# hassony2/homan

Measured on AMD Instinct MI355X. Metric: optimisation iters/sec (30-frame 256^2 clip), higher is better.
Workload: dtype f32

## Files before the change

### homan_amd/csrc/raster_common.h

```cpp
#pragma once
#include "hm_common.h"
#include <type_traits>

#define HM_TILE 8
#define HM_STILE 16
#define RASTER_WAVES 4
#define STAGE_DW 20

typedef int hm_v2i __attribute__((ext_vector_type(2)));
typedef unsigned hm_v4u __attribute__((ext_vector_type(4)));
#ifndef RASTER_NT_STORES
#define RASTER_NT_STORES 0
#endif
__device__ __forceinline__ void hm_out_store(float* p, float v)
{
#if RASTER_NT_STORES
    __builtin_nontemporal_store(v, p);
#else
    *p = v;
#endif
}
__device__ __forceinline__ void hm_out_store2(int* p, int a, int b)
{
#if RASTER_NT_STORES
// ... 14 lines not shown
}

struct FaceBox {
    unsigned short x0m, y0, x1, y1;
};

__device__ __forceinline__ float topix(float v, int is)
{
    float a = v * (float)is;
    a = a + (float)is;
    a = a - 1.0f;
    return 0.5f * a;
}
__device__ __forceinline__ bool backside(const float* f)
{
    return (f[7] - f[1]) * (f[3] - f[0]) < (f[4] - f[1]) * (f[6] - f[0]);
}
__device__ __forceinline__ void wave_sync()
{
    __builtin_amdgcn_fence(__ATOMIC_ACQ_REL, "wavefront");
    __builtin_amdgcn_wave_barrier();
}

#define SR_MAX 64
__host__ __device__ __forceinline__ int hm_sr_shift(int is) { return is <= 512 ? 6 : 7; }

__device__ __forceinline__ int hm_wave_scan_incl(int v)
{
    v += __builtin_amdgcn_update_dpp(0, v, 0x111, 0xf, 0xf, false);
    v += __builtin_amdgcn_update_dpp(0, v, 0x112, 0xf, 0xf, false);
    v += __builtin_amdgcn_update_dpp(0, v, 0x114, 0xf, 0xf, false);
    v += __builtin_amdgcn_update_dpp(0, v, 0x118, 0xf, 0xf, false);
    v += __builtin_amdgcn_update_dpp(0, v, 0x142, 0xa, 0xf, false);
    v += __builtin_amdgcn_update_dpp(0, v, 0x143, 0xc, 0xf, false);
    return v;
}

__device__ __forceinline__ float rlane(float v, int l)
{
    return __builtin_bit_cast(float, __builtin_amdgcn_readlane(__builtin_bit_cast(int, v), l));
}

__device__ __forceinline__ unsigned spread8(unsigned x)
{
    x = (x | (x << 4)) & 0x0f0fu;
    x = (x | (x << 2)) & 0x3333u;
    x = (x | (x << 1)) & 0x5555u;
    return x;
}
__device__ __forceinline__ long hm_plane_at(int b, int ty, int tx, int combo, int T)
{
    return ((((long)b * T + ty) * T + tx) * 4 + combo) * 16;
}
__device__ __forceinline__ unsigned long long hm_plane_word64(const unsigned short* __restrict__ planes, int b, int is,
                                                              int axis, int pl, int d0, int k)
{
    const int T = is / 16;
    unsigned long long w = 0ull;
#pragma unroll
    for (int j = 0; j < 4; ++j) {
        unsigned v;
        if (axis) {
            const int t = is - 1 - d0;
            v = planes[hm_plane_at(b, t >> 4, 4 * k + j, pl, T) + (t & 15)];
        } else {
            v = planes[hm_plane_at(b, T - 1 - (4 * k + j), d0 >> 4, 2 + pl, T) + (d0 & 15)];
        }
        w |= (unsigned long long)v << (16 * j);
    }
    return w;
}
struct Ballots4 { unsigned long long s0, s1, s2, s3; };
__device__ __forceinline__ void emit_planes(const Ballots4 cov, const Ballots4 nb, const Ballots4 pb, int b, int B, int is,
                                            int tx, int ty, int lane, unsigned short* __restrict__ planes)
{
    const int l = lane & 15, pl = (lane >> 4) & 1, hi = l >> 1, sub = l & 1;
    unsigned long long b0, b1;
    unsigned word;
    const Ballots4 g = pl == 0 ? nb : pb;
    if (lane < 32) {
        const unsigned long long c0 = sub ? cov.s2 : cov.s0, c1 = sub ? cov.s3 : cov.s1;
        const unsigned long long g0 = sub ? g.s2 : g.s0, g1 = sub ? g.s3 : g.s1;
        b0 = pl == 0 ? (~c0 & g0) : (c0 & g0);
        b1 = pl == 0 ? (~c1 & g1) : (c1 & g1);
        const unsigned a = (unsigned)(b0 >> (8 * hi)) & 0xffu, o = (unsigned)(b1 >> (8 * hi)) & 0xffu;
        word = spread8(a) | (spread8(o) << 1);
    } else {
        const unsigned long long c0 = sub ? cov.s1 : cov.s0, c1 = sub ? cov.s3 : cov.s2;
        const unsigned long long g0 = sub ? g.s1 : g.s0, g1 = sub ? g.s3 : g.s2;
        b0 = pl == 0 ? (~c0 & g0) : (c0 & g0);
        b1 = pl == 0 ? (~c1 & g1) : (c1 & g1);
        const unsigned k0 = (unsigned)((((b0 >> hi) & 0x0101010101010101ull) * 0x8040201008040201ull) >> 56);
        const unsigned k1 = (unsigned)((((b1 >> hi) & 0x0101010101010101ull) * 0x8040201008040201ull) >> 56);
        word = (spread8(k0) << 1) | spread8(k1);
    }
    const unsigned p2 = (word & 0xffffu) | ((unsigned)__builtin_amdgcn_update_dpp(0, (int)word, 0x101, 0xf, 0xf, false) << 16);
    const unsigned q2 = (unsigned)__builtin_amdgcn_update_dpp(0, (int)p2, 0x102, 0xf, 0xf, false);
    const unsigned r2 = (unsigned)__builtin_amdgcn_update_dpp(0, (int)p2, 0x104, 0xf, 0xf, false);
    const unsigned s2 = (unsigned)__builtin_amdgcn_update_dpp(0, (int)q2, 0x104, 0xf, 0xf, false);
    if ((lane & 7) == 0) hm_out_store4(planes + hm_plane_at(b, ty, tx, 0, is / 16) + lane, p2, q2, r2, s2);
}

__device__ __forceinline__ bool hm_ts_enabled(const unsigned int* __restrict__ flag_word)
{
    return flag_word && ((flag_word[0] >> 8) & 1u);
}
__device__ __forceinline__ void hm_ts_store(unsigned long long* __restrict__ slots, long unit, int which, unsigned long long t)
{
    __builtin_nontemporal_store(t, slots + 2 * unit + which);
}

__device__ __forceinline__ void sil_reduce_frame(int b, const float* __restrict__ partials, int ntiles,
                                                 const float* __restrict__ keep_sum, float* __restrict__ frame_rec,
                                                 float* __restrict__ out, float* __restrict__ frame_out, int clip_len,
                                                 int out_stride)
{
    __shared__ float red[16];
    __shared__ int s_flag;
    float sq = 0.f, in = 0.f, un = 0.f;
    for (int t = threadIdx.x; t < ntiles; t += blockDim.x) {
        const float4 p = *reinterpret_cast<const float4*>(partials + ((long)b * ntiles + t) * 4);
        sq += p.x; in += p.y; un += p.z;
    }
    sq = hm_block_sum(sq, red);
    in = hm_block_sum(in, red);
    un = hm_block_sum(un, red);
    if (threadIdx.x == 0) { hm_partial_store(frame_rec + 4 * b, sq); hm_partial_store(frame_rec + 4 * b + 1, in / (un + 1e-6f)); }
    if (frame_out && threadIdx.x == 0) { frame_out[2 * b] = sq; frame_out[2 * b + 1] = in / (un + 1e-6f); }
    if (!out) return;
    const int clip = b / clip_len;
    float* crec = frame_rec + 4L * clip * clip_len;
    if (hm_last_block(reinterpret_cast<unsigned int*>(crec + 3), clip_len, &s_flag)) {
        const float total_sq = hm_last_block_sum(crec, clip_len, 4, red);
        const float iou_sum = hm_last_block_sum(crec + 1, clip_len, 4, red);
        if (threadIdx.x == 0) {
            out[(long)clip * out_stride] = (total_sq / keep_sum[clip]) / (float)clip_len;
            out[(long)clip * out_stride + 1] = iou_sum / (float)clip_len;
        }
    }
}

struct SweepFace {
    int bf, b, off, flags;
    float px[3], py[3];
    unsigned short cum[12];
};
#define SWEEP_PASS_FACES 16
#ifndef SWEEP_USHIFT
#define SWEEP_USHIFT 8
#endif
#define SWEEP_UNIT (1 << SWEEP_USHIFT)
#define SWEEP_TRIPS (SWEEP_UNIT / 64)
#define SWEEP_TBATCH (SWEEP_TRIPS < 4 ? SWEEP_TRIPS : 4)
struct SweepItem { float x, c0, c1; int base0, base1, nb0, fn, meta; };
struct SweepList {
    SweepFace* tab; int* offs; unsigned int* ufirst; unsigned int* tickets; float* upart;
    unsigned long long* cnt; unsigned int* done; unsigned long long* total;
    int ucap, slot_cap;
};

struct SweepSrc { int d1; float g; int owner; };
#define SWEEP_CUMW 16

template <bool W32> struct HmOff { typedef long t; };
template <> struct HmOff<true> { typedef unsigned t; };
template <bool W32, class T>
__device__ __forceinline__ T* hm_at(T* __restrict__ base, typename HmOff<W32>::t i)
{
    typedef typename std::conditional<std::is_const<T>::value, const char, char>::type byte_t;
    if (W32) return reinterpret_cast<T*>(reinterpret_cast<byte_t*>(base) + (unsigned)(i * (unsigned)sizeof(T)));
    return base + i;
}
```

### homan_amd/csrc/raster_lines.hip

```cpp
#include "raster_ws.h"

__global__ __launch_bounds__(256) void k_bwd_masks(const float* __restrict__ gin, int mode,
                                                   const float* __restrict__ upstream,
                                                   const float* __restrict__ keep_sum, int B, int S,
                                                   const unsigned short* __restrict__ alpha16,
                                                   float* __restrict__ gimg, unsigned short* __restrict__ planes,
                                                   int clip_len)
{
    if (mode == 1 && upstream[0] > 0.0f) return;
    const int w = threadIdx.x >> 6, lane = threadIdx.x & 63;
    const int is = 2 * S, tiles_x = S / HM_TILE, ntiles = tiles_x * tiles_x;
    const int tile = blockIdx.x * 4 + w, b = blockIdx.y;
    if (tile >= ntiles) return;
    const int ty = tile / tiles_x, tx = tile % tiles_x;
    const int rr = lane >> 3, cc = lane & 7;
    const int r = ty * HM_TILE + rr, c = tx * HM_TILE + cc;
    const long po = ((long)b * S + r) * S + c;
    unsigned long long cq[4];
#pragma unroll
    for (int dy = 0; dy < 2; ++dy) {
        const unsigned aw = alpha16[(((long)b * (is / 16) + ty) * (is / 16) + tx) * 16 + 2 * rr + dy];
#pragma unroll
        for (int dx = 0; dx < 2; ++dx) cq[2 * dy + dx] = __ballot((aw >> (2 * cc + dx)) & 1u);
    }
// ... 137 lines not shown
            atomicExch(sl.done, 0u);
        }
    }
}


#ifndef LINES_NL
#define LINES_NL 2
#endif
#ifdef LINES_REVERSED
#define LINES_BLK(i, n) ((n) - 1 - (i))
#else
#define LINES_BLK(i, n) (i)
#endif
template <bool W32>
__global__ __launch_bounds__(256) void k_bwd_lines(const unsigned short* __restrict__ planes,
                                                   const float* __restrict__ gimg, const float* __restrict__ dimg,
                                                   int mode, const float* __restrict__ upstream,
                                                   const float* __restrict__ keep_sum,
                                                   const int* __restrict__ idx_map, int B, int S,
                                                   SweepSrc* __restrict__ srcs, uint4* __restrict__ lrec,
                                                   int ncomp, int fpt, const float* __restrict__ faces9,
                                                   const FaceBox* __restrict__ boxes,
                                                   const unsigned char* __restrict__ owned, int F,
                                                   double* __restrict__ parts, SweepList sl, int clip_len,
                                                   unsigned short* __restrict__ lsum, int nred,
                                                   const float* __restrict__ red_partials, float* __restrict__ frame_rec,
                                                   float* __restrict__ loss_out, int out_stride,
                                                   const unsigned int* __restrict__ ts_flag,
                                                   unsigned long long* __restrict__ ts_slots)
{
    HM_CHAIN_KERNEL();
    const unsigned long long ts_t0 = (unsigned long long)wall_clock64();
    const bool ts_on = hm_ts_enabled(ts_flag) && threadIdx.x == 0;
    if (ts_on) hm_ts_store(ts_slots, blockIdx.x, 0, ts_t0);
    const int blk = (int)blockIdx.x;
    __shared__ unsigned long long s_w[16][LINES_NL][SWEEP_CUMW];
    __shared__ int s_ex[16][LINES_NL][SWEEP_CUMW];
    if (blk < ncomp) {
        sweep_compact(blk, ncomp, fpt, faces9, boxes, owned, B, F, 2 * S, parts, sl, clip_len);
        if (ts_on) hm_ts_store(ts_slots, blockIdx.x, 1, (unsigned long long)wall_clock64());
        return;
    }
    if (blk < ncomp + nred) {
        sil_reduce_frame(blk - ncomp, red_partials, (S / 8) * (S / 8), keep_sum, frame_rec, loss_out, nullptr, clip_len,
                         out_stride);
        if (ts_on) hm_ts_store(ts_slots, blockIdx.x, 1, (unsigned long long)wall_clock64());
        return;
    }
    typedef typename HmOff<W32>::t OFF;
    const int l = threadIdx.x & 15, grp = threadIdx.x >> 4;
    const bool ts_row = l == 0 && hm_ts_enabled(ts_flag);
    const int is = 2 * S, wpl = is / 64, T = is / 16;
    const unsigned Lw = (unsigned)(LINES_BLK(blk - ncomp - nred, (int)gridDim.x - ncomp - nred)) * (16u * LINES_NL);
    const bool valid = Lw < 4u * (unsigned)B * (unsigned)is;
    const unsigned fr = Lw / (unsigned)is;
    const int d00 = (int)(Lw - fr * (unsigned)is) + grp * LINES_NL, b = (int)(fr % (unsigned)B), pa = (int)(fr / (unsigned)B);
    const OFF L0 = (OFF)Lw + (OFF)(grp * LINES_NL);
    const int axis = pa & 1, pl = pa >> 1;
    unsigned long long mine[LINES_NL];
#pragma unroll
    for (int j = 0; j < LINES_NL; ++j) mine[j] = 0ull;
    if (valid && l < wpl) {
        unsigned long long raw[4];
#pragma unroll
        for (int jj = 0; jj < 4; ++jj) {
            OFF at;
            if (axis) {
                const int t = is - 1 - d00 - (LINES_NL - 1);
                at = ((((OFF)b * T + (t >> 4)) * T + (4 * l + jj)) * 4 + pl) * 16 + (t & 15);
            } else {
                at = ((((OFF)b * T + (T - 1 - (4 * l + jj))) * T + (d00 >> 4)) * 4 + (2 + pl)) * 16 + (d00 & 15);
            }
#if LINES_NL == 4
            raw[jj] = *reinterpret_cast<const unsigned long long*>(hm_at<W32>(planes, at));
#elif LINES_NL == 2
            raw[jj] = *reinterpret_cast<const unsigned int*>(hm_at<W32>(planes, at));
#else
            raw[jj] = *hm_at<W32>(planes, at);
#endif
        }
#pragma unroll
        for (int j = 0; j < LINES_NL; ++j) {
            const int sel = axis ? LINES_NL - 1 - j : j;
#pragma unroll
            for (int jj = 0; jj < 4; ++jj) mine[j] |= ((raw[jj] >> (16 * sel)) & 0xffffull) << (16 * jj);
        }
    }
    bool any = false;
#pragma unroll
    for (int j = 0; j < LINES_NL; ++j) {
        const OFF L = L0 + j;
        const int d0 = d00 + j;
        const int c = __popcll(mine[j]);
        int incl = c;
        incl += __builtin_amdgcn_update_dpp(0, incl, 0x111, 0xf, 0xf, false);
        incl += __builtin_amdgcn_update_dpp(0, incl, 0x112, 0xf, 0xf, false);
        incl += __builtin_amdgcn_update_dpp(0, incl, 0x114, 0xf, 0xf, false);
        incl += __builtin_amdgcn_update_dpp(0, incl, 0x118, 0xf, 0xf, false);
        const int excl = incl - c;
        if (valid && l < wpl) *hm_at<W32>(lrec, L * wpl + l) = make_uint4((unsigned)mine[j], (unsigned)(mine[j] >> 32), (unsigned)excl, 0u);
        int lo = mine[j] ? 64 * l + __builtin_ctzll(mine[j]) : 0xffff, hi = mine[j] ? 64 * l + 64 - __builtin_clzll(mine[j]) : 0;
        lo = min(lo, __builtin_amdgcn_update_dpp(0xffff, lo, 0x111, 0xf, 0xf, false)); hi = max(hi, __builtin_amdgcn_update_dpp(0, hi, 0x111, 0xf, 0xf, false));
        lo = min(lo, __builtin_amdgcn_update_dpp(0xffff, lo, 0x112, 0xf, 0xf, false)); hi = max(hi, __builtin_amdgcn_update_dpp(0, hi, 0x112, 0xf, 0xf, false));
        lo = min(lo, __builtin_amdgcn_update_dpp(0xffff, lo, 0x114, 0xf, 0xf, false)); hi = max(hi, __builtin_amdgcn_update_dpp(0, hi, 0x114, 0xf, 0xf, false));
        lo = min(lo, __builtin_amdgcn_update_dpp(0xffff, lo, 0x118, 0xf, 0xf, false)); hi = max(hi, __builtin_amdgcn_update_dpp(0, hi, 0x118, 0xf, 0xf, false));
        const unsigned wm = (unsigned)(__ballot(mine[j] != 0ull) >> (16 * (grp & 3))) & 0xffffu;
        if (valid && l == 15)
            *reinterpret_cast<uint2*>(hm_at<W32>(lsum, ((((OFF)b * 2 + axis) * is + d0) * 2 + pl) * 4)) =
                make_uint2((unsigned)lo | ((unsigned)hi << 16), wm);
        any = any || wm != 0u;
        s_w[grp][j][l] = mine[j];
        s_ex[grp][j][l] = excl;
    }
    wave_sync();
    if (!valid || !any) {
        if (ts_row) atomicMax(ts_slots + 2 * blockIdx.x + 1, (unsigned long long)wall_clock64());
        return;
    }
    const bool from_dimg = mode == 2 || (mode == 1 && upstream[0] > 0.0f);
    const float* gi = (from_dimg ? dimg : gimg) + (long)b * S * S;
    const float gs = from_dimg ? upstream[0] * 2.0f : 0.f, ks = from_dimg ? keep_sum[b / clip_len] : 1.f;
    const float up4 = (mode == 4 || mode == 5) ? upstream[b] * 2.0f : 0.f;
    const int* idx = idx_map + (long)b * is * is;
    const float* gfull = gimg + (long)b * is * is;
#pragma unroll 1
    for (int j = 0; j < LINES_NL; ++j) {
        const int d0 = d00 + j;
        const OFF out0 = (L0 + j) * is;
        for (int k = 0; k < wpl; ++k) {
            const unsigned long long w = s_w[grp][j][k];
            if (w == 0ull) continue;
            const int base = s_ex[grp][j][k];
            float gl[4];
            int ow[4];
#pragma unroll
            for (int q = 0; q < 4; ++q) {
                const int pos = 16 * q + l;
                gl[q] = 0.f;
                ow[q] = -1;
                if (!((w >> pos) & 1ull)) continue;
                const int d1 = (k << 6) + pos;
                const int xi = axis ? d1 : d0, yi = axis ? d0 : d1;
                if (mode == 5) gl[q] = pl ? 1.0f : -1.0f;
                else if (mode == 3 || mode == 4) gl[q] = gfull[(is - 1 - yi) * is + xi];
                else gl[q] = gi[((is - 1 - yi) >> 1) * S + (xi >> 1)];
                if (pl) ow[q] = idx[yi * is + xi];
            }
#pragma unroll
            for (int q = 0; q < 4; ++q) {
                const int pos = 16 * q + l;
                if (!((w >> pos) & 1ull)) continue;
                SweepSrc r;
                r.d1 = (k << 6) + pos;
                float g = gl[q];
                if (mode == 4 || mode == 5) g = up4 * g;
                else if (mode != 3) {
                    if (from_dimg) g = gs * g / ks / (float)clip_len;
                    g = 0.25f * g;
                }
                r.g = g;
                r.owner = ow[q];
                *hm_at<W32>(srcs, out0 + (OFF)(base + __popcll(w & ((1ull << pos) - 1ull)))) = r;
            }
        }
    }
    if (ts_row) atomicMax(ts_slots + 2 * blockIdx.x + 1, (unsigned long long)wall_clock64());
}

void hm_launch_bwd_masks(const SilWs& w, const float* gin, int mode, const float* upstream, const float* keep_sum, int B, int S,
                         int clip_len, hipStream_t stream)
{
    const int ntiles = (S / 8) * (S / 8);
    hipLaunchKernelGGL(k_bwd_masks, dim3(hm_cdiv(ntiles, 4), B), dim3(256), 0, stream, gin, mode, upstream, keep_sum, B, S,
                       w.alpha16, w.gimg, w.planes, clip_len);
}
void hm_launch_lines(const SilWs& w, int B, int F, int S, int mode, const float* upstream, const float* keep_sum, int clip_len,
                     hipStream_t stream, float* loss_out, int out_stride)
{
    const int nred = loss_out ? B : 0;
    const int fpt = (long)clip_len * F >= 400000 ? 4 : 1;
    const int ncomp = (B / clip_len) * hm_cdiv((long)clip_len * F, 256 * fpt);
    const bool w32 = hm_offsets_fit_32(B, S);
    hipLaunchKernelGGL(w32 ? k_bwd_lines<true> : k_bwd_lines<false>, dim3(ncomp + nred + hm_cdiv(4L * B * 2 * S, 16 * LINES_NL)), dim3(256), 0, stream, w.planes,
                       w.gimg, w.dimg, mode, upstream, keep_sum, w.idx_map, B, S, w.srcs, w.lrec, ncomp, fpt, w.faces9, w.boxes,
                       w.owned, F, w.parts, w.sweep, clip_len, w.lsum, nred, w.partials, w.frame_rec, loss_out, out_stride,
                       w.counter + 24, w.ts + 2 * ts_raster_units(B, S));
}
```

### homan_amd/csrc/raster_sweep.hip

```cpp
#include "raster_ws.h"
#include "raster_hooks.h"

__device__ __forceinline__ float sample_grad(const float* __restrict__ gimg, int S, int is, int xi, int yi)
{
    return 0.25f * gimg[(long)((is - 1 - yi) >> 1) * S + (xi >> 1)];
}

__device__ __forceinline__ void sweep_term(float diff, int d1, float d1_cross, float k0, float k1, bool use0, bool use1,
                                           float eps, double magic, double& acc0, double& acc1)
{
    const float t = (float)d1 - d1_cross;
    const bool live = diff > 0.0f;
    float dist0 = k0 * t, dist1 = k1 * t;
    dist0 += (0.0f < dist0) ? eps : -eps;
    dist1 += (0.0f < dist1) ? eps : -eps;
    const float g0 = diff / dist0, g1 = diff / dist1;
    acc0 -= hm_quant((live && use0) ? g0 : 0.0f, magic);
    acc1 -= hm_quant((live && use1) ? g1 : 0.0f, magic);
}
__device__ __forceinline__ float sweep_item_scale(float c, float two_over_is, bool pow2, int is)
{
    return pow2 ? (c * 2.0f) * two_over_is : (c * 2.0f) / (float)is;
}

__device__ __forceinline__ void raster_reorder(int* __restrict__ wo_dyn, int* __restrict__ wo_tmp,
                                               const unsigned int* __restrict__ wg_cost, unsigned int* __restrict__ dyn_flag, int n,
                                               unsigned* __restrict__ s_hist)
{
    __shared__ unsigned s_wsum[4];
    __shared__ unsigned s_zero;
    const int tid = threadIdx.x, lane = tid & 63, wv = tid >> 6;
    for (int i = tid; i < 1024; i += 256) s_hist[i] = 0u;
    if (tid == 0) s_zero = 0u;
    __syncthreads();
    for (int base = 0; base < n; base += 256 * 16) {
        unsigned cv[16];
#pragma unroll
        for (int k = 0; k < 16; ++k) { const int i = base + 256 * k + tid; cv[k] = i < n ? wg_cost[i] : 0u; }
#pragma unroll
        for (int k = 0; k < 16; ++k)
            if (base + 256 * k + tid < n && cv[k] != 0u) atomicAdd(&s_hist[1023 - min(cv[k] >> 2, 1023u)], 1u);
    }
    __syncthreads();
    unsigned c[4], tot = 0u;
#pragma unroll
    for (int k = 0; k < 4; ++k) { c[k] = s_hist[4 * tid + k]; tot += c[k]; }
    const unsigned incl = (unsigned)hm_wave_scan_incl((int)tot);
    if (lane == 63) s_wsum[wv] = incl;
    __syncthreads();
    unsigned base0 = incl - tot;
    for (int q = 0; q < wv; ++q) base0 += s_wsum[q];
    const unsigned n_busy = s_wsum[0] + s_wsum[1] + s_wsum[2] + s_wsum[3];
#pragma unroll
    for (int k = 0; k < 4; ++k) { s_hist[4 * tid + k] = base0; base0 += c[k]; }
    __syncthreads();
    for (int base = 0; base < n; base += 256 * 16) {
        unsigned cv[16];
        int ev[16];
#pragma unroll
        for (int k = 0; k < 16; ++k) {
            const int i = base + 256 * k + tid;
            cv[k] = i < n ? wg_cost[i] : 0u;
            ev[k] = i < n ? wo_dyn[i] : 0;
        }
#pragma unroll
        for (int k = 0; k < 16; ++k) {
            const bool in = base + 256 * k + tid < n, zero = in && cv[k] == 0u;
            const unsigned long long zb = __ballot(zero);
            unsigned zbase = 0u;
            if (lane == 0 && zb) zbase = atomicAdd(&s_zero, (unsigned)__popcll(zb));
            zbase = (unsigned)__builtin_amdgcn_readfirstlane((int)zbase);
            if (zero) wo_tmp[n_busy + zbase + (unsigned)__popcll(zb & ((1ull << lane) - 1ull))] = ev[k];
            else if (in) wo_tmp[atomicAdd(&s_hist[1023 - min(cv[k] >> 2, 1023u)], 1u)] = ev[k];
        }
    }
    __threadfence();
    __syncthreads();
    for (int base = 0; base < n; base += 256 * 16) {
        int ev[16];
#pragma unroll
        for (int k = 0; k < 16; ++k) { const int i = base + 256 * k + tid; ev[k] = i < n ? __builtin_nontemporal_load(wo_tmp + i) : 0; }
#pragma unroll
        for (int k = 0; k < 16; ++k) { const int i = base + 256 * k + tid; if (i < n) wo_dyn[i] = ev[k]; }
    }
    if (tid == 0) *dyn_flag = 1u;
}

#ifdef SWEEP_STATS
__device__ unsigned long long g_sweep_n[16];
#endif
#ifdef SWEEP_UNIT_PROFILE
__device__ int g_unit_prof[65536][4];
#endif
struct SweepGeo {
    int var, edge, axis, d0r, dir, a_in, a_out;
    float p00, p01, p10, p11, p20, p21, num, d1_cross;
    bool geo;
};
struct SweepLite { int var, axis, d0r, a_in, a_out; bool geo, pos; };
__device__ __forceinline__ SweepLite sweep_item_lite(const SweepFace& fc, const int2* __restrict__ famtab, int j, bool mine, int is)
{
    SweepLite q;
    int fam = 0;
#pragma unroll
    for (int stp = 8; stp > 0; stp >>= 1)
        if ((int)fc.cum[fam + stp - 1] <= j) fam += stp;
    const int fstart = fam ? (int)fc.cum[fam - 1] : 0;
    q.var = fam >= 6 ? 1 : 0;
    const int ci = fam - 6 * q.var;
    q.axis = ci & 1;
    const int edge = ci >> 1, v0 = q.var ? 2 - edge : edge;
    const float p00 = (q.axis ? fc.py : fc.px)[v0], p01 = (q.axis ? fc.px : fc.py)[v0];
    const int2 ft = famtab[fam];
    const float slope = __int_as_float(ft.x);
    const bool lt = (ft.y >> 16) & 1;
    const int dir = q.axis == 0 ? (lt ? -1 : 1) : (lt ? 1 : -1);
    q.d0r = mine ? (ft.y & 0xffff) + (j - fstart) : 0;
    const float d1_cross = slope * ((float)q.d0r - p00) + p01;
    bool geo = mine && d1_cross > -8.0f && d1_cross < (float)is + 8.0f;
    const int d1_in = geo ? ((dir > 0) ? (int)floorf(d1_cross) : (int)ceilf(d1_cross)) : 0;
    const int d1_out = d1_in + dir;
    geo = geo && !(d1_in < 0 || is <= d1_in || d1_out < 0 || is <= d1_out);
    q.a_in = geo ? d1_in : 0;
    q.a_out = geo ? d1_out : 0;
    q.geo = geo;
    q.pos = dir > 0;
    return q;
}
__device__ __forceinline__ SweepGeo sweep_item_geo(const SweepFace& fc, int j, bool mine, int is,
                                                   const int2* __restrict__ famtab = nullptr)
{
    SweepGeo q;
    int fam = 0;
#pragma unroll
    for (int stp = 8; stp > 0; stp >>= 1)
        if ((int)fc.cum[fam + stp - 1] <= j) fam += stp;
    const int fstart = fam ? (int)fc.cum[fam - 1] : 0;
    q.var = fam >= 6 ? 1 : 0;
    const int ci = fam - 6 * q.var;
    q.edge = ci >> 1;
    q.axis = ci & 1;
    int v0 = q.edge, v1 = q.edge == 2 ? 0 : q.edge + 1, v2 = q.edge == 0 ? 2 : q.edge - 1;
    if (q.var) { v0 = 2 - v0; v1 = 2 - v1; v2 = 2 - v2; }
    const float* pa = q.axis ? fc.py : fc.px;
    const float* pb = q.axis ? fc.px : fc.py;
    q.p00 = pa[v0]; q.p01 = pb[v0]; q.p10 = pa[v1]; q.p11 = pb[v1]; q.p20 = pa[v2]; q.p21 = pb[v2];
    if (q.axis == 0) q.dir = (q.p00 < q.p10) ? -1 : 1;
    else q.dir = (q.p00 < q.p10) ? 1 : -1;
    const int d0_from = (int)fmaxf(ceilf(fminf(q.p00, q.p10)), 0.0f);
    q.num = q.p10 - q.p00;
    const float slope = famtab ? __int_as_float(famtab[fam].x) : (q.p11 - q.p01) / q.num;
    q.d0r = mine ? d0_from + (j - fstart) : 0;
    q.d1_cross = slope * ((float)q.d0r - q.p00) + q.p01;
    bool geo = mine && q.d1_cross > -8.0f && q.d1_cross < (float)is + 8.0f;
    const int d1_in = geo ? ((q.dir > 0) ? (int)floorf(q.d1_cross) : (int)ceilf(q.d1_cross)) : 0;
    const int d1_out = d1_in + q.dir;
    geo = geo && !(d1_in < 0 || is <= d1_in || d1_out < 0 || is <= d1_out);
    q.a_in = geo ? d1_in : 0;
    q.a_out = geo ? d1_out : 0;
    q.geo = geo;
    return q;
}

#ifndef SWEEP_COMBINE_MIN
#define SWEEP_COMBINE_MIN 32
#endif
#ifndef SWEEP_COMBINE_PAIRS
#define SWEEP_COMBINE_PAIRS 192
#endif
__device__ __forceinline__ double sweep_row_sum(double v)
{
    v += hm_dpp_f64<0xb1, 0xf>(v);
    v += hm_dpp_f64<0x4e, 0xf>(v);
    v += hm_dpp_f64<0x114, 0xf>(v);
    v += hm_dpp_f64<0x118, 0xf>(v);
    return v;
}
__device__ __forceinline__ void sweep_combine_rows(int& cur, double& acc0, double& acc1, bool flush, int lane)
{
    const unsigned long long nb = __ballot(flush);
    if (__popcll(nb) < SWEEP_COMBINE_MIN) return;
    const int prev = __builtin_amdgcn_update_dpp(cur, cur, 0x111, 0xf, 0xf, false);
    const unsigned long long same = __ballot(prev == cur);
    const int sh = lane & 48;
    const bool uni = ((unsigned)(nb >> sh) & (unsigned)(same >> sh) & 0xffffu) == 0xffffu;
    const double r0 = sweep_row_sum(acc0), r1 = sweep_row_sum(acc1);
    if (uni) {
        if ((lane & 15) == 15) { acc0 = r0; acc1 = r1; }
        else { cur = -1; acc0 = 0.0; acc1 = 0.0; }
    }
}

#ifndef SWEEP_WAVES_EU
#define SWEEP_WAVES_EU 5
#endif
template <bool W32>
__global__ __launch_bounds__(256) __attribute__((amdgpu_waves_per_eu(SWEEP_WAVES_EU, 8))) void k_bwd_sweep(SweepList sl, const int* __restrict__ idx_map,
                                                   const SweepSrc* __restrict__ srcs,
                                                   const uint4* __restrict__ lrec, int B, int F, int S,
                                                   float eps, double magic, double* __restrict__ parts,
                                                   const unsigned short* __restrict__ lsum,
                                                   const unsigned short* __restrict__ alpha16,
                                                   const unsigned int* __restrict__ ts_flag,
                                                   unsigned long long* __restrict__ ts_slots, int nsort,
                                                   int* __restrict__ wo_dyn, int* __restrict__ wo_tmp,
                                                   const unsigned int* __restrict__ wg_cost,
                                                   unsigned int* __restrict__ dyn_flag, int n_wo)
{
    HM_CHAIN_KERNEL();
    typedef typename HmOff<W32>::t OFF;
    const unsigned long long ts_t0 = (unsigned long long)wall_clock64();
    const bool ts_on = hm_ts_enabled(ts_flag) && (threadIdx.x & 63) == 0;
    if (ts_on) hm_ts_store(ts_slots, (long)blockIdx.x * 4 + (threadIdx.x >> 6), 0, ts_t0);
    struct FaceLds { SweepFace f; int pad; };
    struct ItemLds { SweepItem it; int pad; };
    __shared__ FaceLds s_face[4][SWEEP_PASS_FACES];
    __shared__ double s_fg[4][SWEEP_PASS_FACES][6];
    __shared__ int s_start[4][64];
    __shared__ int s_head[4][256];
    __shared__ ItemLds s_item[4][64];
    __shared__ unsigned short s_q[4][SWEEP_UNIT];
    __shared__ int2 s_fam[4][SWEEP_PASS_FACES][12];
    __shared__ int s_fb[4][SWEEP_PASS_FACES][2];
    if (nsort && blockIdx.x == 0) {
        raster_reorder(wo_dyn, wo_tmp, wg_cost, dyn_flag, n_wo, reinterpret_cast<unsigned*>(&s_head[0][0]));
        if (ts_on) hm_ts_store(ts_slots, (long)blockIdx.x * 4 + (threadIdx.x >> 6), 1, (unsigned long long)wall_clock64());
        return;
    }
    const int wid = (int)blockIdx.x - nsort, nwork = (int)gridDim.x - nsort;
    const int lane = threadIdx.x & 63, wv = threadIdx.x >> 6;
    const int is = 2 * S;
    const bool pow2 = (is & (is - 1)) == 0;
    const float inv_is = 1.0f / (float)is;
    const int wpl = is / 64;
    const unsigned long long tot = sl.total[0];
    const int N = (int)(tot & 0xffffffffull), W = (int)(tot >> 32);
    const int U = (N + SWEEP_UNIT - 1) >> SWEEP_USHIFT;
    const int xcd = wid & 7;
    const int xwaves = (nwork >> 3) * 4;
    const int u_end = (int)(((long)U * (xcd + 1)) >> 3);
    int first_ahead = -1;
    for (int u = __builtin_amdgcn_readfirstlane((int)(((long)U * xcd) >> 3) + (wid >> 3) * 4 + wv); u < u_end;
         u += xwaves) {
        const int ubeg = u << SWEEP_USHIFT, uend = ubeg + SWEEP_UNIT;
#ifdef SWEEP_UNIT_PROFILE
        const unsigned long long up_t0 = wall_clock64();
        int up_pass = 0, up_trips = 0, up_q = 0, up_rounds = 0;
#endif
        int first = first_ahead;
        if (first < 0) {
            if (u < sl.ucap) first = (int)sl.ufirst[u];
            else {
                int lo = 0, hi = W - 1;
                while (lo < hi) {
                    const int mid = (lo + hi + 1) >> 1;
                    if (sl.offs[mid] <= ubeg) lo = mid; else hi = mid - 1;
                }
                first = lo;
            }
            first = __builtin_amdgcn_readfirstlane(first);
        }
        const int u_ahead = u + xwaves;
        int ahead_v = -1;
        if (u_ahead < u_end && u_ahead < sl.ucap) ahead_v = (int)sl.ufirst[u_ahead];
        for (int fb = 0;; fb += SWEEP_PASS_FACES) {
            const int o = (lane <= SWEEP_PASS_FACES && first + fb + lane < W) ? sl.offs[first + fb + lane] : 0x7fffffff;
            int row[SWEEP_PASS_FACES / 4];
#pragma unroll
            for (int k = 0; k < SWEEP_PASS_FACES / 4; ++k) {
                const int fi = first + fb + 4 * k + (lane >> 4);
                row[k] = fi < W ? reinterpret_cast<const int*>(sl.tab + fi)[lane & 15] : 0;
            }
            if (fb == 0) first_ahead = __builtin_amdgcn_readfirstlane(ahead_v);
            const int nfp = __popcll(__ballot(lane < SWEEP_PASS_FACES && o < uend));
            if (nfp == 0) break;
#ifdef SWEEP_UNIT_PROFILE
            ++up_pass;
#endif
            const int it_lo = max(ubeg, __builtin_amdgcn_readlane(o, 0));
            const int it_hi = min(min(uend, N), __builtin_amdgcn_readlane(o, nfp));
            __builtin_amdgcn_wave_barrier();
#pragma unroll
            for (int k = 0; k < SWEEP_PASS_FACES / 4; ++k) {
                const int ent = 4 * k + (lane >> 4);
                if (ent < nfp) reinterpret_cast<int*>(&s_face[wv][ent].f)[lane & 15] = row[k];
            }
            for (int i = lane; i < SWEEP_PASS_FACES * 6; i += 64) (&s_fg[wv][0][0])[i] = 0.0;
            wave_sync();
            for (int idx = lane; idx < nfp * 12; idx += 64) {
                const int e = idx / 12, fam = idx - 12 * e;
                const SweepFace& f = s_face[wv][e].f;
                const int var = fam >= 6 ? 1 : 0, ci = fam - 6 * var, edge = ci >> 1, axis = ci & 1;
                int v0 = edge, v1 = edge == 2 ? 0 : edge + 1;
                if (var) { v0 = 2 - v0; v1 = 2 - v1; }
                const float* pa = axis ? f.py : f.px;
                const float* pb = axis ? f.px : f.py;
                const float p00 = pa[v0], p10 = pa[v1], p01 = pb[v0], p11 = pb[v1];
                const float slope = (p11 - p01) / (p10 - p00);
                const int d0_from = (int)fmaxf(ceilf(fminf(p00, p10)), 0.0f);
                s_fam[wv][e][fam] = make_int2(__float_as_int(slope), (d0_from & 0xffff) | ((p00 < p10) ? 1 << 16 : 0));
            }
            if (lane < 2 * nfp) {
                const int e = lane >> 1, axis = lane & 1;
                const SweepFace& f = s_face[wv][e].f;
                const float* pb = axis ? f.px : f.py;
                const float tmin = fminf(pb[0], fminf(pb[1], pb[2])), tmax = fmaxf(pb[0], fmaxf(pb[1], pb[2]));
                s_fb[wv][e][axis] = max(0, (int)floorf(fmaxf(tmin, 0.f)) - 1) | (min(is - 1, (int)ceilf(fminf(tmax, (float)is)) + 1) << 16);
            }
            wave_sync();
            SWEEP_HOOK_PASS_STAGED(eps, nfp);
            int qn = 0;
            {
              for (int tb = 0; tb < SWEEP_TRIPS; tb += SWEEP_TBATCH) {
                uint4 sm[SWEEP_TBATCH];
                int s_io[SWEEP_TBATCH], s_lohi[SWEEP_TBATCH], s_ent[SWEEP_TBATCH], s_own[SWEEP_TBATCH], s_fn[SWEEP_TBATCH];
                unsigned short s_aw[SWEEP_TBATCH];
#pragma unroll
                for (int t = 0; t < SWEEP_TBATCH; ++t) {
                    const int g = it_lo + 64 * (tb + t) + lane;
                    int el = -1;
                    for (int i = 0; i < nfp; ++i) el += (__builtin_amdgcn_readlane(o, i) <= g) ? 1 : 0;
                    const SweepFace& fc = s_face[wv][max(el, 0)].f;
                    const bool mine = g < it_hi && el >= 0 && g - fc.off < (int)fc.cum[11];
                    const SweepLite q = sweep_item_lite(fc, s_fam[wv][max(el, 0)], mine ? g - fc.off : 0, mine, is);
                    sm[t] = *reinterpret_cast<const uint4*>(hm_at<W32>(lsum, (((OFF)fc.b * 2 + q.axis) * is + q.d0r) * 8));
                    {
                        const int xi_in = q.axis ? q.a_in : q.d0r, yi_in = q.axis ? q.d0r : q.a_in;
                        const int xi_out = q.axis ? q.a_out : q.d0r, yo = is - 1 - (q.axis ? q.d0r : q.a_out);
                        s_own[t] = *hm_at<W32>(idx_map, ((OFF)fc.b * is + yi_in) * is + xi_in);
                        s_aw[t] = *hm_at<W32>(alpha16, ((((OFF)fc.b * (is >> 4)) + (yo >> 4)) * (is >> 4) + (xi_out >> 4)) * 16 + (yo & 15));
                        s_aw[t] = (unsigned short)((s_aw[t] >> (xi_out & 15)) & 1u);
                        s_fn[t] = fc.bf - fc.b * F + q.var * F;
                    }
                    s_io[t] = q.a_in | (q.pos ? 1 << 12 : 0) | (q.geo ? 1 << 13 : 0);
                    {
                        const int fbv = s_fb[wv][max(el, 0)][q.axis];
                        s_lohi[t] = q.pos ? ((fbv & 0xffff) | (q.a_in << 16)) : (q.a_in | (fbv & 0xffff0000));
                    }
                    s_ent[t] = (g - ubeg) | (max(el, 0) << SWEEP_USHIFT);
                }
#pragma unroll
                for (int t = 0; t < SWEEP_TBATCH; ++t) {
                    const int min0 = (int)(sm[t].x & 0xffffu), end0 = (int)(sm[t].x >> 16);
                    const int min1 = (int)(sm[t].z & 0xffffu), end1 = (int)(sm[t].z >> 16);
                    const bool pos = (s_io[t] >> 12) & 1, geo_t = (s_io[t] >> 13) & 1;
                    const int a_in_t = s_io[t] & 0xfff, a_out_t = a_in_t + (pos ? 1 : -1);
                    const int lo_t = s_lohi[t] & 0xffff, hi_t = s_lohi[t] >> 16;
                    const bool out_ok = pos ? end0 > a_out_t : min0 <= a_out_t;
                    const int wlo = lo_t >> 6, whi = hi_t >> 6;
                    const bool in_ok = lo_t <= hi_t && min1 <= hi_t && end1 > lo_t &&
                                       ((sm[t].w >> wlo) & ((2u << (whi - wlo)) - 1u)) != 0u;
                    const bool a0 = geo_t && s_own[t] == s_fn[t] && out_ok;
                    const bool a1 = geo_t && s_aw[t] == 0 && in_ok;
                    const bool reach = a0 || a1;
                    const unsigned long long bal = __ballot(reach);
#ifdef SWEEP_STATS
                    const unsigned long long gbal = __ballot(geo_t);
                    if (lane == 0) {
                        atomicAdd(&g_sweep_n[8], (unsigned long long)max(0, min(64, it_hi - (it_lo + 64 * (tb + t)))));
                        atomicAdd(&g_sweep_n[9], (unsigned long long)__popcll(gbal));
                        atomicAdd(&g_sweep_n[10], (unsigned long long)__popcll(bal));
                    }
                    {
                        const unsigned long long b12 = __ballot(geo_t && s_own[t] == s_fn[t]), b13 = __ballot(a0);
                        const unsigned long long b14 = __ballot(geo_t && s_aw[t] == 0), b15 = __ballot(a1);
                        if (lane == 0) {
                            atomicAdd(&g_sweep_n[12], (unsigned long long)__popcll(b12)); atomicAdd(&g_sweep_n[13], (unsigned long long)__popcll(b13));
                            atomicAdd(&g_sweep_n[14], (unsigned long long)__popcll(b14)); atomicAdd(&g_sweep_n[15], (unsigned long long)__popcll(b15));
                        }
                    }
#endif
                    if (reach) s_q[wv][qn + __popcll(bal & ((1ull << lane) - 1ull))] =
                                   (unsigned short)(s_ent[t] | (a0 ? 1 << 14 : 0) | (a1 ? 1 << 15 : 0));
                    qn += __popcll(bal);
                }
              }
            }
            wave_sync();
            SWEEP_HOOK_STAGE1_DONE(eps, qn);
#ifdef SWEEP_UNIT_PROFILE
            up_q += qn;
#endif
            for (int s0 = 0; s0 < qn; s0 += 64) {
#ifdef SWEEP_UNIT_PROFILE
            ++up_trips;
#endif
            bool mine = s0 + lane < qn;
            const int ent = mine ? (int)s_q[wv][s0 + lane] : 0;
            const int g = ubeg + (ent & (SWEEP_UNIT - 1)), el = (ent >> SWEEP_USHIFT) & 15;
            const SweepFace& fc = s_face[wv][el].f;
            const SweepGeo q = sweep_item_geo(fc, mine ? g - fc.off : 0, mine, is, s_fam[wv][el]);
            const int var = q.var, edge = q.edge, axis = q.axis, d0r = q.d0r, dir = q.dir, a_in = q.a_in, a_out = q.a_out;
            const float p00 = q.p00, p01 = q.p01, p10 = q.p10, p11 = q.p11, p20 = q.p20, p21 = q.p21, num = q.num;
            const float d1_cross = q.d1_cross;
            const bool geo = q.geo;
            const int b = fc.b, fn = fc.bf - b * F + var * F;
            const bool use0 = p10 != (float)d0r, use1 = p00 != (float)d0r;
            const float c0 = use0 ? num / (p10 - (float)d0r) : 0.f;
            const float c1 = use1 ? num / ((float)d0r - p00) : 0.f;
            const bool act0 = geo && (ent & (1 << 14));
            const bool act1 = geo && (ent & (1 << 15));
            int rfrom[2], rto[2];
            {
                const int lim = (dir > 0) ? is - 1 : 0;
                rfrom[0] = max(min(a_out, lim), 0);
                rto[0] = min(max(a_out, lim), is - 1);
            }
            rfrom[1] = 0;
            rto[1] = -1;
            if (act1) {
                const bool far02 = ((float)d0r - p00) * ((float)d0r - p20) < 0.0f;
                const float na = far02 ? p21 - p01 : p11 - p21, da = far02 ? p20 - p00 : p10 - p20;
                const float ba = far02 ? p00 : p20, oa = far02 ? p01 : p21;
                float c2 = na / da * ((float)d0r - ba) + oa;
                if (c2 == c2) {
                    c2 = fminf(fmaxf(c2, -4.0f), (float)is + 4.0f);
                    const int lim = (dir > 0) ? (int)ceilf(c2) : (int)floorf(c2);
                    rfrom[1] = max(min(a_in, lim), 0);
                    rto[1] = min(max(a_in, lim), is - 1);
                }
            }
            const bool on[2] = {act0 && rfrom[0] <= rto[0], act1 && rfrom[1] <= rto[1]};
            int lo[2] = {0, 0}, nbp[2] = {0, 0};
            OFF lid[2];
            uint4 rf[2], rt[2];
#pragma unroll
            for (int ph = 0; ph < 2; ++ph) {
                lid[ph] = ((OFF)(ph * 2 + axis) * B + b) * is + d0r;
                rf[ph] = make_uint4(0u, 0u, 0u, 0u);
                rt[ph] = rf[ph];
                if (on[ph]) {
                    rf[ph] = *hm_at<W32>(lrec, lid[ph] * wpl + (rfrom[ph] >> 6));
                    rt[ph] = *hm_at<W32>(lrec, lid[ph] * wpl + (rto[ph] >> 6));
                }
            }
#pragma unroll
            for (int ph = 0; ph < 2; ++ph) {
                const unsigned long long wf = rf[ph].x | ((unsigned long long)rf[ph].y << 32);
                const unsigned long long wt = rt[ph].x | ((unsigned long long)rt[ph].y << 32);
                lo[ph] = (int)rf[ph].z + __popcll(wf & ((1ull << (rfrom[ph] & 63)) - 1ull));
                nbp[ph] = on[ph] ? (int)rt[ph].z + __popcll(wt & (~0ull >> (63 - (rto[ph] & 63)))) - lo[ph] : 0;
            }
            const int nb0 = nbp[0], nb1 = nbp[1];
#ifdef SWEEP_STATS
            {
                const unsigned long long c[7] = {__popcll(__ballot(mine)), __popcll(__ballot(geo)), __popcll(__ballot(act0)),
                                                 __popcll(__ballot(act1)), __popcll(__ballot(nb0 > 0)), __popcll(__ballot(nb1 > 0)),
                                                 (unsigned long long)hm_wave_scan_incl(nb0 + nb1)};
                if (lane == 63) { for (int k = 0; k < 7; ++k) atomicAdd(&g_sweep_n[k], c[k]); atomicAdd(&g_sweep_n[7], 1ull); }
            }
#endif
            const int n = nb0 + nb1;
            const int incl = hm_wave_scan_incl(n);
            const int npairs = __builtin_amdgcn_readlane(incl, 63);
            if (npairs > 0) {
                __builtin_amdgcn_wave_barrier();
                s_start[wv][lane] = incl - n;
                SweepItem it;
                it.x = d1_cross;
                it.c0 = sweep_item_scale(c0, inv_is, pow2, is);
                it.c1 = sweep_item_scale(c1, inv_is, pow2, is);
                it.base0 = (int)(lid[0] * is) + lo[0];
                it.base1 = (int)(lid[1] * is) + lo[1];
                it.nb0 = nb0;
                it.fn = fn;
                {
                    const int m0 = var ? 2 - edge : edge, k1 = edge == 2 ? 0 : edge + 1, m1 = var ? 2 - k1 : k1;
                    const int comp = axis ? 0 : 1;
                    it.meta = el | ((2 * m0 + comp) << 4) | ((2 * m1 + comp) << 7) | (use0 ? 1 << 10 : 0) |
                              (use1 ? 1 << 11 : 0) | (nb0 << 12);
                }
                s_item[wv][lane].it = it;
                wave_sync();
                const int* st = s_start[wv];
                int cur = -1;
                double acc0 = 0.0, acc1 = 0.0;
                int carry = 0;
#pragma unroll 1
                for (int base = 0; base < npairs; base += 256) {
                    SWEEP_HOOK_PAIR_ROUND(eps, base);
#ifdef SWEEP_STATS
                    if (lane == 0) atomicAdd(&g_sweep_n[11], 1ull);
#endif
#ifdef SWEEP_UNIT_PROFILE
                    ++up_rounds;
#endif
                    int4* hd = reinterpret_cast<int4*>(s_head[wv]);
                    hd[lane] = make_int4(0, 0, 0, 0);
                    wave_sync();
                    const int ex = incl - n;
                    if (n > 0 && ex >= base && ex < base + 256) s_head[wv][ex - base] = lane + 1;
                    wave_sync();
                    const int4 h = hd[lane];
                    int m[4];
                    m[0] = h.x; m[1] = max(m[0], h.y); m[2] = max(m[1], h.z); m[3] = max(m[2], h.w);
                    int inc = m[3];
                    inc = max(inc, __builtin_amdgcn_update_dpp(0, inc, 0x111, 0xf, 0xf, false));
                    inc = max(inc, __builtin_amdgcn_update_dpp(0, inc, 0x112, 0xf, 0xf, false));
                    inc = max(inc, __builtin_amdgcn_update_dpp(0, inc, 0x114, 0xf, 0xf, false));
                    inc = max(inc, __builtin_amdgcn_update_dpp(0, inc, 0x118, 0xf, 0xf, false));
                    inc = max(inc, __builtin_amdgcn_update_dpp(0, inc, 0x142, 0xa, 0xf, false));
                    inc = max(inc, __builtin_amdgcn_update_dpp(0, inc, 0x143, 0xc, 0xf, false));
                    int before = __builtin_amdgcn_update_dpp(0, inc, 0x138, 0xf, 0xf, false);
                    before = max(before, carry);
                    carry = max(carry, __builtin_amdgcn_readlane(inc, 63));
                    SweepSrc sc[4];
                    int qi[4], qmeta[4];
                    bool ph1[4];
#pragma unroll
                    for (int k = 0; k < 4; ++k) {
                        const int p = min(base + 4 * lane + k, npairs - 1);
                        const int i = max(max(before, m[k]) - 1, 0);
                        const int r = max(p - st[i], 0);
                        const SweepItem& qq = s_item[wv][i].it;
                        qmeta[k] = qq.meta;
                        const int q_nb0 = qmeta[k] >> 12;
                        ph1[k] = r >= q_nb0;
                        qi[k] = i;
                        OFF at = (OFF)qq.base0 + r;
                        if (ph1[k]) at = (OFF)qq.base1 + (r - q_nb0);
                        sc[k] = *hm_at<W32>(srcs, at);
                    }
#if SWEEP_COMBINE_MIN <= 64
                    if (base > 0) {
                        const int key0 = base + 4 * lane < npairs ? (qmeta[0] & 0x3ff) : cur;
                        sweep_combine_rows(cur, acc0, acc1, cur >= 0 && key0 != cur, lane);
                    }
#endif
#pragma unroll
                    for (int k = 0; k < 4; ++k) {
                        {
                            const bool valid = base + 4 * lane + k < npairs;
                            const SweepItem& qq = s_item[wv][qi[k]].it;
                            const int meta = qmeta[k], key = valid ? (meta & 0x3ff) : cur;
                            if (key != cur) {
                                if (cur >= 0) {
#ifdef SWEEP_HOOK_FLUSH
                                    SWEEP_HOOK_FLUSH(eps, s_fg[wv], lane, cur, acc0, acc1);
#else
                                    double* f = s_fg[wv][cur & 15];
                                    unsafeAtomicAdd(f + ((cur >> 4) & 7), acc0);
                                    unsafeAtomicAdd(f + ((cur >> 7) & 7), acc1);
#endif
                                }
                                cur = key;
                                acc0 = 0.0;
                                acc1 = 0.0;
                            }
                            const bool take = valid && (!ph1[k] || sc[k].owner == qq.fn);
                            sweep_term(take ? (ph1[k] ? sc[k].g : -sc[k].g) : 0.0f, sc[k].d1, qq.x, qq.c0, qq.c1,
                                       (meta & (1 << 10)) != 0, (meta & (1 << 11)) != 0, eps, magic, acc0, acc1);
                        }
                    }
                }
#if SWEEP_COMBINE_MIN <= 64
                if (npairs >= SWEEP_COMBINE_PAIRS) sweep_combine_rows(cur, acc0, acc1, cur >= 0, lane);
#endif
                if (cur >= 0) {
                    double* f = s_fg[wv][cur & 15];
                    unsafeAtomicAdd(f + ((cur >> 4) & 7), acc0);
                    unsafeAtomicAdd(f + ((cur >> 7) & 7), acc1);
                }
            }
            wave_sync();
            }
            if (lane < nfp) {
                const SweepFace& ff = s_face[wv][lane].f;
                const int off = ff.off, nit = (int)ff.cum[11];
                const int u_lo = off >> SWEEP_USHIFT, u_hi = (off + nit - 1) >> SWEEP_USHIFT;
                double v[6];
#pragma unroll
                for (int k = 0; k < 6; ++k) v[k] = s_fg[wv][lane][k];
                double* out = parts + (long)ff.bf * 6;
                if (u_lo == u_hi) {
#pragma unroll
                    for (int k = 0; k < 6; ++k) out[k] = v[k];
                } else {
#pragma unroll
                    for (int k = 0; k < 6; ++k) unsafeAtomicAdd(out + k, v[k]);
                }
            }
            if (nfp < SWEEP_PASS_FACES) break;
        }
#ifdef SWEEP_UNIT_PROFILE
        if (lane == 0 && u < 65536) {
            g_unit_prof[u][0] = (int)(wall_clock64() - up_t0); g_unit_prof[u][1] = up_pass;
            g_unit_prof[u][2] = up_trips | (up_q << 8); g_unit_prof[u][3] = up_rounds;
        }
#endif
    }
    if (ts_on) hm_ts_store(ts_slots, (long)blockIdx.x * 4 + (threadIdx.x >> 6), 1, (unsigned long long)wall_clock64());
}

__global__ void k_bwd_gather(const double* __restrict__ parts, const int* __restrict__ adj_off,
                             const int* __restrict__ adj_items, const float* __restrict__ verts,
                             const float* __restrict__ K, int B, int V, int F, float orig_size,
                             float* __restrict__ grad_ndc, float* __restrict__ grad_verts)
{
    const long i = (long)blockIdx.x * blockDim.x + threadIdx.x;
    if (i >= (long)B * V) return;
    const int b = (int)(i / V), v = (int)(i % V);
    double su = 0.0, sv = 0.0;
    const double2* pf = reinterpret_cast<const double2*>(parts + (long)b * F * 6);
    const int a1 = adj_off[v + 1];
    for (int a = adj_off[v]; a < a1; a += 8) {
        int item[8];
#pragma unroll
        for (int k = 0; k < 8; ++k) item[k] = a + k < a1 ? adj_items[a + k] : -1;
        double2 g2[8];
#pragma unroll
        for (int k = 0; k < 8; ++k) g2[k] = item[k] >= 0 ? pf[item[k]] : make_double2(0.0, 0.0);
#pragma unroll
        for (int k = 0; k < 8; ++k) { su += g2[k].x; sv += g2[k].y; }
    }
    const float gu = (float)su, gv = (float)sv;
    if (grad_ndc) { grad_ndc[3 * i] = gu; grad_ndc[3 * i + 1] = gv; grad_ndc[3 * i + 2] = 0.f; }
    const float* k = K + b * 9;
    const float x = verts[3 * i], y = verts[3 * i + 1], z = verts[3 * i + 2];
    const float zz = z + 1e-9f;
    const float du0 = gu * (2.0f / orig_size), dv0 = -gv * (2.0f / orig_size);
    const float dxn = k[0] * du0 + k[3] * dv0;
    const float dyn = k[1] * du0 + k[4] * dv0;
    grad_verts[3 * i] = dxn / zz;
    grad_verts[3 * i + 1] = dyn / zz;
    grad_verts[3 * i + 2] = -(dxn * x + dyn * y) / (zz * zz);
}

void hm_launch_sweep(const SilWs& w, int B, int F, int S, float eps, int sum_log2q, hipStream_t stream)
{
    const RasterTune& tune = hm_raster_tune();
    const int nsort = tune.raster_reorder ? 1 : 0;
    const int blocks = max(8, (min(min(hm_cdiv((long)B * F, 2), tune.sweep_blocks), TS_SWEEP_WGS - 8) & ~7) - 8 * nsort);
    const bool w32 = hm_offsets_fit_32(B, S);
    hipLaunchKernelGGL(w32 ? k_bwd_sweep<true> : k_bwd_sweep<false>, dim3(nsort + blocks), dim3(256), 0, stream, w.sweep,
                       w.idx_map, w.srcs, w.lrec, B, F, S, eps, hm_sum_magic(sum_log2q), w.parts, w.lsum, w.alpha16, w.counter + 24,
                       w.ts + 2 * (ts_raster_units(B, S) + ts_lines_units(B, F, S)), nsort, w.wo_dyn, w.wo_tmp, w.wg_cost,
                       w.counter + 26, (int)ts_raster_units(B, S));
}
void hm_launch_bwd_gather(const SilWs& w, const int* adj_off, const int* adj_items, const float* verts, const float* K, int B,
                          int V, int F, float orig_size, float* grad_ndc, float* grad_verts, hipStream_t stream)
{
    hipLaunchKernelGGL(k_bwd_gather, dim3(hm_cdiv((long)B * V, 256)), dim3(256), 0, stream, w.parts, adj_off, adj_items, verts,
                       K, B, V, F, orig_size, grad_ndc, grad_verts);
}
int hm_sweep_occupancy(int* blocks_per_cu)
{
    return hipOccupancyMaxActiveBlocksPerMultiprocessor(blocks_per_cu, k_bwd_sweep<true>, 256, 0) == hipSuccess ? HM_OK : HM_ERR_LAUNCH;
}
#ifdef SWEEP_UNIT_PROFILE
extern "C" int hm_debug_unit_profile(int* out)
{
    (void)hipDeviceSynchronize();
    (void)hipMemcpyFromSymbol(out, HIP_SYMBOL(g_unit_prof), sizeof(int) * 65536 * 4);
    static int z[65536][4];
    (void)hipMemcpyToSymbol(HIP_SYMBOL(g_unit_prof), z, sizeof(z));
    return HM_OK;
}
#endif
#ifdef SWEEP_STATS
extern "C" int hm_debug_sweep_stats(unsigned long long* out)
{
    unsigned long long z[16] = {0, 0, 0, 0, 0, 0, 0, 0, 0, 0, 0, 0, 0, 0, 0, 0};
    (void)hipDeviceSynchronize();
    (void)hipMemcpyFromSymbol(out, HIP_SYMBOL(g_sweep_n), sizeof(z));
    (void)hipMemcpyToSymbol(HIP_SYMBOL(g_sweep_n), z, sizeof(z));
    return HM_OK;
}
#endif
```

Before: 6612.

## Repack sweep items and sources to simplify pair-to-source address math

SweepItem is repacked into a 16-byte-aligned struct with precomputed byte-offset bases and a split point, so each pair's source address takes one compare and one add instead of a lookup of the start index and several subtractions. The separate start array is removed and two int4/float4 LDS reads replace the field-by-field loads. The source records now store d1 as a float and the gradient with its sign already applied and clamped to zero, which removes the int-to-float conversion and the live-flag select. The use0/use1 flags move into the high bits of meta and are applied with bit masks, which adds dependence on that packing and on the gradient sign folding being equivalent to the old code.

```diff
diff --git a/homan_amd/csrc/raster_common.h b/homan_amd/csrc/raster_common.h
--- a/homan_amd/csrc/raster_common.h
+++ b/homan_amd/csrc/raster_common.h
@@ -190,14 +190,14 @@
 #define SWEEP_UNIT (1 << SWEEP_USHIFT)
 #define SWEEP_TRIPS (SWEEP_UNIT / 64)
 #define SWEEP_TBATCH (SWEEP_TRIPS < 4 ? SWEEP_TRIPS : 4)
-struct SweepItem { float x, c0, c1; int base0, base1, nb0, fn, meta; };
+struct alignas(16) SweepItem { int baseA, split, meta, baseB; float x, c0, c1; int fn; };
 struct SweepList {
     SweepFace* tab; int* offs; unsigned int* ufirst; unsigned int* tickets; float* upart;
     unsigned long long* cnt; unsigned int* done; unsigned long long* total;
     int ucap, slot_cap;
 };
 
-struct SweepSrc { int d1; float g; int owner; };
+struct SweepSrc { float d1; float g; int owner; };
 #define SWEEP_CUMW 16
 
 template <bool W32> struct HmOff { typedef long t; };
diff --git a/homan_amd/csrc/raster_lines.hip b/homan_amd/csrc/raster_lines.hip
--- a/homan_amd/csrc/raster_lines.hip
+++ b/homan_amd/csrc/raster_lines.hip
@@ -313,14 +313,15 @@
                 const int pos = 16 * q + l;
                 if (!((w >> pos) & 1ull)) continue;
                 SweepSrc r;
-                r.d1 = (k << 6) + pos;
+                r.d1 = (float)((k << 6) + pos);
                 float g = gl[q];
                 if (mode == 4 || mode == 5) g = up4 * g;
                 else if (mode != 3) {
                     if (from_dimg) g = gs * g / ks / (float)clip_len;
                     g = 0.25f * g;
                 }
-                r.g = g;
+                const float gd = pl ? g : -g;
+                r.g = gd > 0.0f ? gd : 0.0f;
                 r.owner = ow[q];
                 *hm_at<W32>(srcs, out0 + (OFF)(base + __popcll(w & ((1ull << pos) - 1ull)))) = r;
             }
diff --git a/homan_amd/csrc/raster_sweep.hip b/homan_amd/csrc/raster_sweep.hip
--- a/homan_amd/csrc/raster_sweep.hip
+++ b/homan_amd/csrc/raster_sweep.hip
@@ -6,17 +6,17 @@
     return 0.25f * gimg[(long)((is - 1 - yi) >> 1) * S + (xi >> 1)];
 }
 
-__device__ __forceinline__ void sweep_term(float diff, int d1, float d1_cross, float k0, float k1, bool use0, bool use1,
+__device__ __forceinline__ void sweep_term(float diff, float d1, float d1_cross, float k0, float k1, int meta,
                                            float eps, double magic, double& acc0, double& acc1)
 {
-    const float t = (float)d1 - d1_cross;
-    const bool live = diff > 0.0f;
+    const float t = d1 - d1_cross;
     float dist0 = k0 * t, dist1 = k1 * t;
     dist0 += (0.0f < dist0) ? eps : -eps;
     dist1 += (0.0f < dist1) ? eps : -eps;
-    const float g0 = diff / dist0, g1 = diff / dist1;
-    acc0 -= hm_quant((live && use0) ? g0 : 0.0f, magic);
-    acc1 -= hm_quant((live && use1) ? g1 : 0.0f, magic);
+    const float n0 = __int_as_float(__float_as_int(diff) & ((int)((unsigned)meta << 1) >> 31));
+    const float n1 = __int_as_float(__float_as_int(diff) & ((int)((unsigned)meta << 2) >> 31));
+    acc0 -= hm_quant(n0 / dist0, magic);
+    acc1 -= hm_quant(n1 / dist1, magic);
 }
 __device__ __forceinline__ float sweep_item_scale(float c, float two_over_is, bool pow2, int is)
 {
@@ -213,12 +213,10 @@
     const bool ts_on = hm_ts_enabled(ts_flag) && (threadIdx.x & 63) == 0;
     if (ts_on) hm_ts_store(ts_slots, (long)blockIdx.x * 4 + (threadIdx.x >> 6), 0, ts_t0);
     struct FaceLds { SweepFace f; int pad; };
-    struct ItemLds { SweepItem it; int pad; };
     __shared__ FaceLds s_face[4][SWEEP_PASS_FACES];
     __shared__ double s_fg[4][SWEEP_PASS_FACES][6];
-    __shared__ int s_start[4][64];
     __shared__ int s_head[4][256];
-    __shared__ ItemLds s_item[4][64];
+    __shared__ SweepItem s_item[4][65];
     __shared__ unsigned short s_q[4][SWEEP_UNIT];
     __shared__ int2 s_fam[4][SWEEP_PASS_FACES][12];
     __shared__ int s_fb[4][SWEEP_PASS_FACES][2];
@@ -455,24 +453,24 @@
             const int npairs = __builtin_amdgcn_readlane(incl, 63);
             if (npairs > 0) {
                 __builtin_amdgcn_wave_barrier();
-                s_start[wv][lane] = incl - n;
+                const int ps = W32 ? (int)sizeof(SweepSrc) : 1;
+                const int st0 = incl - n;
                 SweepItem it;
                 it.x = d1_cross;
                 it.c0 = sweep_item_scale(c0, inv_is, pow2, is);
                 it.c1 = sweep_item_scale(c1, inv_is, pow2, is);
-                it.base0 = (int)(lid[0] * is) + lo[0];
-                it.base1 = (int)(lid[1] * is) + lo[1];
-                it.nb0 = nb0;
+                it.baseA = (int)(((unsigned)(lid[0] * is) + (unsigned)(lo[0] - st0)) * (unsigned)ps);
+                it.split = (st0 + nb0) * ps;
+                it.baseB = (int)(((unsigned)(lid[1] * is) + (unsigned)(lo[1] - (st0 + nb0))) * (unsigned)ps);
                 it.fn = fn;
                 {
                     const int m0 = var ? 2 - edge : edge, k1 = edge == 2 ? 0 : edge + 1, m1 = var ? 2 - k1 : k1;
                     const int comp = axis ? 0 : 1;
-                    it.meta = el | ((2 * m0 + comp) << 4) | ((2 * m1 + comp) << 7) | (use0 ? 1 << 10 : 0) |
-                              (use1 ? 1 << 11 : 0) | (nb0 << 12);
-                }
-                s_item[wv][lane].it = it;
+                    it.meta = el | ((2 * m0 + comp) << 4) | ((2 * m1 + comp) << 7) | (use1 ? 1 << 29 : 0) | (use0 ? 1 << 30 : 0);
+                }
+                s_item[wv][lane + 1] = it;
                 wave_sync();
-                const int* st = s_start[wv];
+                const int plast = (npairs - 1) * ps;
                 int cur = -1;
                 double acc0 = 0.0, acc1 = 0.0;
                 int carry = 0;
@@ -507,33 +505,32 @@
                     SweepSrc sc[4];
                     int qi[4], qmeta[4];
                     bool ph1[4];
+                    const int pp0 = (base + 4 * lane) * ps;
 #pragma unroll
                     for (int k = 0; k < 4; ++k) {
-                        const int p = min(base + 4 * lane + k, npairs - 1);
-                        const int i = max(max(before, m[k]) - 1, 0);
-                        const int r = max(p - st[i], 0);
-                        const SweepItem& qq = s_item[wv][i].it;
-                        qmeta[k] = qq.meta;
-                        const int q_nb0 = qmeta[k] >> 12;
-                        ph1[k] = r >= q_nb0;
+                        const int pp = min(pp0 + k * ps, plast);
+                        const int i = max(max(before, m[k]), 1);
+                        const int4 a = *reinterpret_cast<const int4*>(&s_item[wv][i]);
+                        qmeta[k] = a.z;
+                        ph1[k] = pp >= a.y;
                         qi[k] = i;
-                        OFF at = (OFF)qq.base0 + r;
-                        if (ph1[k]) at = (OFF)qq.base1 + (r - q_nb0);
-                        sc[k] = *hm_at<W32>(srcs, at);
+                        const int ab = ph1[k] ? a.w : a.x;
+                        if (W32) sc[k] = *reinterpret_cast<const SweepSrc*>(reinterpret_cast<const char*>(srcs) + ((unsigned)ab + (unsigned)pp));
+                        else sc[k] = srcs[(long)ab + pp];
                     }
 #if SWEEP_COMBINE_MIN <= 64
                     if (base > 0) {
-                        const int key0 = base + 4 * lane < npairs ? (qmeta[0] & 0x3ff) : cur;
+                        const int key0 = base + 4 * lane < npairs ? qmeta[0] : cur;
                         sweep_combine_rows(cur, acc0, acc1, cur >= 0 && key0 != cur, lane);
                     }
 #endif
 #pragma unroll
                     for (int k = 0; k < 4; ++k) {
                         {
-                            const bool valid = base + 4 * lane + k < npairs;
-                            const SweepItem& qq = s_item[wv][qi[k]].it;
-                            const int meta = qmeta[k], key = valid ? (meta & 0x3ff) : cur;
-                            if (key != cur) {
+                            const bool valid = base + 4 * lane < npairs - k;
+                            const float4 tq = *reinterpret_cast<const float4*>(&s_item[wv][qi[k]].x);
+                            const int meta = qmeta[k];
+                            if (valid && meta != cur) {
                                 if (cur >= 0) {
 #ifdef SWEEP_HOOK_FLUSH
                                     SWEEP_HOOK_FLUSH(eps, s_fg[wv], lane, cur, acc0, acc1);
@@ -543,13 +540,12 @@
                                     unsafeAtomicAdd(f + ((cur >> 7) & 7), acc1);
 #endif
                                 }
-                                cur = key;
+                                cur = meta;
                                 acc0 = 0.0;
                                 acc1 = 0.0;
                             }
-                            const bool take = valid && (!ph1[k] || sc[k].owner == qq.fn);
-                            sweep_term(take ? (ph1[k] ? sc[k].g : -sc[k].g) : 0.0f, sc[k].d1, qq.x, qq.c0, qq.c1,
-                                       (meta & (1 << 10)) != 0, (meta & (1 << 11)) != 0, eps, magic, acc0, acc1);
+                            const bool take = valid && (!ph1[k] || sc[k].owner == __float_as_int(tq.w));
+                            sweep_term(take ? sc[k].g : 0.0f, sc[k].d1, tq.x, tq.y, tq.z, meta, eps, magic, acc0, acc1);
                         }
                     }
                 }
```

Result: faster. 6686 (median of 6 runs) (+1.1%).
